# kjedrzejewski/video-cycle_gan-upscaling

Measured on AMD Instinct MI355X. Metric: upscaled frames/s (train step, G+D fwd+bwd) at 256->512, higher is better.
Workload: dtype f32; 1 GPU; C2: make_upscaler_orig((512,512,3),k=3,x2,res=9) + PatchGAN-70, batch 8/GPU, gan2 wiring, Wasserstein + pixel-MSE, faithful 3-call step incl. predict pass; global_batch=8, frame=256x256->512x512, parallelism=dp1, launch=hipGraph replay

## Files before the change

video-cycle_gan-upscaling_amd/csrc/conv_fwd.hip:

```cpp
#include "vcg_common.hpp"
#include <type_traits>

namespace {

struct ConvParams {
    const float* x;
    const float* w;
    float* y;
    const float* bias;
    const float* prelu;
    const float* residual;
    int n, cin, h, w_, cout, oh, ow, pad_top, pad_left;
    int tiles_x, tiles_y, co_blocks;
    int act;
    float alpha;
    int flip;
    int ws_t, ws_m, ws_k;
    float* stats;
};

template <int KH, int KW, int S, int CK, int XT>
struct ConvCfg {
    static constexpr int ROWS = 8;
    static constexpr int IH = (ROWS - 1) * S + KH;
    static constexpr int IW = (32 * XT - 1) * S + KW;
    static constexpr int PLANE = IH * IW;
    static constexpr int T = KH * KW;
    static constexpr int IN_ELEMS = CK * PLANE;
    static constexpr int W_ELEMS = CK * T * 64;
    static constexpr int IN_PT = (IN_ELEMS + 255) / 256;
    static constexpr int W_PT = (W_ELEMS + 255) / 256;
    static constexpr size_t LDS_BYTES = (size_t)(IN_ELEMS + W_ELEMS) * sizeof(float);
};

template <int XT>
__device__ __forceinline__ void conv_epilogue(const ConvParams& p, f32x16 (&acc)[2][2][XT], int n, int co0, int oy0, int ox0,
                                              int wv, int lane) {
    const int half = lane >> 5, l31 = lane & 31;
    const unsigned plane = (unsigned)(p.oh * p.ow), plane4 = 4u * plane, ow4 = 4u * (unsigned)p.ow;
    const int nch = p.cout - co0 < 64 ? p.cout - co0 : 64;
    const size_t blk = ((size_t)n * p.cout + co0) * plane;
    const size_t blk_bytes = (size_t)nch * plane * sizeof(float);
    const vcg_rsrc ry = make_rsrc(p.y + blk, blk_bytes);
    const vcg_rsrc rr = make_rsrc(p.residual ? p.residual + blk : nullptr, p.residual ? blk_bytes : 0);
    const bool is_prelu = p.act == VCG_ACT_PRELU;
    const vcg_rsrc rbias = make_rsrc(p.bias, p.bias ? (size_t)p.cout * sizeof(float) : 0);
    const vcg_rsrc rslope = make_rsrc(is_prelu ? p.prelu : nullptr, is_prelu ? (size_t)p.cout * sizeof(float) : 0);
    const float slope_u = (p.act == VCG_ACT_LRELU) ? p.alpha : 1.f;
    const unsigned chan4 = 4u * (unsigned)(co0 + 4 * half);

    const int oy = oy0 + wv * 2, ox = ox0 + l31;
    const unsigned base = (unsigned)(4 * half) * plane4 + (unsigned)oy * ow4 + 4u * (unsigned)ox;
    unsigned vo[2][XT];
#pragma unroll
    for (int rt = 0; rt < 2; ++rt)
#pragma unroll
        for (int xt = 0; xt < XT; ++xt)
            vo[rt][xt] = (oy + rt < p.oh && ox + xt * 32 < p.ow) ? base + (unsigned)rt * ow4 + 128u * xt : VCG_OOB;

    constexpr int RG = 8 / XT, NG = 32 / RG;
    auto emit = [&](auto res_tag) {
        constexpr bool RES = decltype(res_tag)::value;
        float rs[2][RG][2][XT];
        auto row_of = [](int g, int j) { const int q = g * RG + j, r = q & 15; return (q >> 4) * 32 + (r & 3) + 8 * (r >> 2); };
        auto load_res = [&](int g) {
#pragma unroll
            for (int j = 0; j < RG; ++j) {
                const unsigned srow = (unsigned)row_of(g, j) * plane4;
#pragma unroll
                for (int rt = 0; rt < 2; ++rt)
#pragma unroll
                    for (int xt = 0; xt < XT; ++xt) rs[g & 1][j][rt][xt] = buf_load(rr, __builtin_elementwise_add_sat(vo[rt][xt], srow));
            }
        };
        if (RES) load_res(0);
#pragma unroll
        for (int g = 0; g < NG; ++g) {
            float bv[RG], al[RG];
#pragma unroll
            for (int j = 0; j < RG; ++j) {
                bv[j] = buf_load(rbias, chan4 + 4u * (unsigned)row_of(g, j));
                const float pa = buf_load(rslope, chan4 + 4u * (unsigned)row_of(g, j));
                al[j] = is_prelu ? pa : slope_u;
            }
            if (RES && g + 1 < NG) load_res(g + 1);
#pragma unroll
            for (int j = 0; j < RG; ++j) {
                const int q = g * RG + j;
                const unsigned srow = (unsigned)row_of(g, j) * plane4;
#pragma unroll
                for (int rt = 0; rt < 2; ++rt) {
#pragma unroll
                    for (int xt = 0; xt < XT; ++xt) {
                        float v = acc[q >> 4][rt][xt][q & 15] + bv[j];
                        v = v >= 0.f ? v : v * al[j];
                        if (RES) v += rs[g & 1][j][rt][xt];
                        buf_store(ry, __builtin_elementwise_add_sat(vo[rt][xt], srow), v);
                    }
                }
            }
        }
    };
    if (p.residual) emit(std::true_type{}); else emit(std::false_type{});
}

template <int XT>
__device__ __forceinline__ void conv_stats_epilogue(const ConvParams& p, f32x16 (&acc)[2][2][XT], float* smem, int rec, int co0, int oy0, int ox0,
                                                    int wv, int lane, int tid) {
    const int half = lane >> 5, l31 = lane & 31;
    float sv[32], sq[32];
#pragma unroll
    for (int mt = 0; mt < 2; ++mt)
#pragma unroll
        for (int r = 0; r < 16; ++r) {
            float a = 0.f, b = 0.f;
#pragma unroll
            for (int rt = 0; rt < 2; ++rt)
#pragma unroll
                for (int xt = 0; xt < XT; ++xt) {
                    const bool ok = oy0 + wv * 2 + rt < p.oh && ox0 + l31 + xt * 32 < p.ow;
                    const float v = ok ? acc[mt][rt][xt][r] : 0.f;
                    a += v;
                    b = fmaf(v, v, b);
                }
            sv[mt * 16 + r] = a;
            sq[mt * 16 + r] = b;
        }
    const float ts = half_wave_reduce_scatter32(sv, l31), tq = half_wave_reduce_scatter32(sq, l31);
    const int ch = (l31 >> 4) * 32 + (l31 & 3) + 8 * ((l31 & 15) >> 2) + 4 * half;
    __syncthreads();
    smem[(0 * 4 + wv) * 64 + ch] = ts;
    smem[(1 * 4 + wv) * 64 + ch] = tq;
    __syncthreads();
    if (tid < 128) {
        const int st = tid >> 6, c = tid & 63;
        const float t = (smem[(st * 4 + 0) * 64 + c] + smem[(st * 4 + 1) * 64 + c]) + (smem[(st * 4 + 2) * 64 + c] + smem[(st * 4 + 3) * 64 + c]);
        if (co0 + c < p.cout) p.stats[((size_t)rec * 2 + st) * p.cout + co0 + c] = t;
    }
}

template <int KH, int KW, int S, int CK, int XT, bool STATS = false>
__global__ __launch_bounds__(256, (KH >= 9 ? 1 : 2)) void conv_fwd_kernel(const ConvParams p) {
    using C = ConvCfg<KH, KW, S, CK, XT>;
    extern __shared__ __attribute__((aligned(16))) float smem[];
    float* s_in = smem;
    float* s_w = smem + C::IN_ELEMS;

    const int tid = threadIdx.x, lane = tid & 63, wv = tid >> 6;
    const int half = lane >> 5, l31 = lane & 31;
    int b = blockIdx.x;
    const int cb = b % p.co_blocks; b /= p.co_blocks;
    const int tx = b % p.tiles_x;   b /= p.tiles_x;
    const int ty = b % p.tiles_y;   b /= p.tiles_y;
    const int n = b;
    const int ox0 = tx * 32 * XT, oy0 = ty * C::ROWS, co0 = cb * 64;
    const int gy0 = oy0 * S - p.pad_top, gx0 = ox0 * S - p.pad_left;
    const float* xn = p.x + (size_t)n * p.cin * p.h * p.w_;

    float rin[C::IN_PT], rw[C::W_PT];

    const int hw = p.h * p.w_;
    const int wvu = __builtin_amdgcn_readfirstlane(wv);
    const unsigned wcol = 4u * (unsigned)(co0 + lane < p.cout ? co0 + lane : p.cout - 1);
    const size_t wbytes = (size_t)C::T * p.cin * p.cout * sizeof(float);

    auto in_rsrc = [&](int ci0) { return make_rsrc(xn + (size_t)ci0 * hw, (size_t)(p.cin - ci0) * hw * sizeof(float)); };
    auto load_w = [&](int ci0) {
        const vcg_rsrc rwt = make_rsrc(p.w + (size_t)ci0 * p.cout, wbytes - (size_t)ci0 * p.cout * sizeof(float));
#pragma unroll
        for (int i = 0; i < C::W_PT; ++i) {
            const int q = wvu + 4 * i;
            const int t = q % C::T, ci = q / C::T;
            const int tap = p.flip ? (C::T - 1 - t) : t;
            rw[i] = buf_load(rwt, 4u * (unsigned)((tap * p.cin + ci) * p.cout) + wcol);
        }
    };
    load_w(0);
    __builtin_amdgcn_sched_barrier(0);

    unsigned in_off[C::IN_PT];
    {
        constexpr int Q1 = 256 / C::PLANE, R1 = 256 % C::PLANE, QR = R1 / C::IW, RC = R1 % C::IW;
        const vcg_rsrc rx = in_rsrc(0);
        const unsigned w4 = 4u * (unsigned)p.w_, hw4 = 4u * (unsigned)hw;
        const unsigned step = (unsigned)Q1 * hw4 + (unsigned)QR * w4 + 4u * RC;
        const unsigned col_wrap = w4 - 4u * C::IW, row_wrap = hw4 - (unsigned)C::IH * w4;
        int ci = tid / C::PLANE, r = (tid % C::PLANE) / C::IW, c = (tid % C::PLANE) % C::IW;
        unsigned off = (unsigned)ci * hw4 + (unsigned)(gy0 + r) * w4 + 4u * (unsigned)(gx0 + c);
#pragma unroll
        for (int i = 0; i < C::IN_PT; ++i) {
            const bool in_tile = (i + 1) * 256 <= C::IN_ELEMS || ci < CK;
            const bool ok = in_tile && (unsigned)(gy0 + r) < (unsigned)p.h && (unsigned)(gx0 + c) < (unsigned)p.w_;
            in_off[i] = ok ? off : VCG_OOB;
            rin[i] = buf_load(rx, in_off[i]);
            __builtin_amdgcn_sched_barrier(0);
            c += RC;
            const bool cw = c >= C::IW;
            c -= cw ? C::IW : 0;
            r += QR + (cw ? 1 : 0);
            const bool rwr = r >= C::IH;
            r -= rwr ? C::IH : 0;
            ci += Q1 + (rwr ? 1 : 0);
            off += step + (cw ? col_wrap : 0u) + (rwr ? row_wrap : 0u);
        }
    }
    auto load_chunk = [&](int ci0) {
        const vcg_rsrc rx = in_rsrc(ci0);
#pragma unroll
        for (int i = 0; i < C::IN_PT; ++i) rin[i] = buf_load(rx, in_off[i]);
        load_w(ci0);
    };
    auto store_chunk = [&]() {
#pragma unroll
        for (int i = 0; i < C::IN_PT; ++i) {
            const int e = tid + i * 256;
            if (e < C::IN_ELEMS) s_in[e] = rin[i];
        }
#pragma unroll
        for (int i = 0; i < C::W_PT; ++i) {
            const int e = tid + i * 256;
            if (e < C::W_ELEMS) s_w[e] = rw[i];
        }
    };

    f32x16 acc[2][2][XT];
#pragma unroll
    for (int i = 0; i < 2; ++i)
#pragma unroll
        for (int j = 0; j < 2; ++j)
#pragma unroll
            for (int x = 0; x < XT; ++x)
#pragma unroll
                for (int r = 0; r < 16; ++r) acc[i][j][x][r] = 0.f;

    const float* bbase = s_in + half * C::PLANE + (wv * 2 * S) * C::IW + l31 * S;
    const float* abase = s_w + half * C::T * 64 + l31;

    const int nchunks = (p.cin + CK - 1) / CK;
    for (int c = 0; c < nchunks; ++c) {
        __syncthreads();
        store_chunk();
        __syncthreads();
        if (c + 1 < nchunks) load_chunk((c + 1) * CK);
        constexpr int NTAP = (CK / 2) * C::T;
        auto rd = [&](int q, float (&a)[2], float (&b)[2][XT]) {
            const int cp = q / C::T, t = q % C::T, ky = t / KW, kx = t % KW;
            a[0] = abase[(cp * 2 * C::T + t) * 64];
            a[1] = abase[(cp * 2 * C::T + t) * 64 + 32];
#pragma unroll
            for (int xt = 0; xt < XT; ++xt) {
                b[0][xt] = bbase[cp * 2 * C::PLANE + ky * C::IW + kx + xt * 32 * S];
                b[1][xt] = bbase[cp * 2 * C::PLANE + (S + ky) * C::IW + kx + xt * 32 * S];
            }
        };
        float a_[2][2], b_[2][2][XT];
        rd(0, a_[0], b_[0]);
#pragma unroll
        for (int q = 0; q < NTAP; ++q) {
            const int cur = q & 1, nxt = cur ^ 1;
            if (q + 1 < NTAP) rd(q + 1, a_[nxt], b_[nxt]);
#pragma unroll
            for (int xt = 0; xt < XT; ++xt) {
                acc[0][0][xt] = mfma32(a_[cur][0], b_[cur][0][xt], acc[0][0][xt]);
                acc[0][1][xt] = mfma32(a_[cur][0], b_[cur][1][xt], acc[0][1][xt]);
                acc[1][0][xt] = mfma32(a_[cur][1], b_[cur][0][xt], acc[1][0][xt]);
                acc[1][1][xt] = mfma32(a_[cur][1], b_[cur][1][xt], acc[1][1][xt]);
            }
            if (q + 1 < NTAP) __builtin_amdgcn_sched_group_barrier(0x100, 1 + 2 * XT, 0);
            __builtin_amdgcn_sched_group_barrier(0x008, 4 * XT, 0);
        }
    }

    conv_epilogue<XT>(p, acc, n, co0, oy0, ox0, wv, lane);
    if (STATS) conv_stats_epilogue<XT>(p, acc, smem, (n * p.tiles_y + ty) * p.tiles_x + tx, co0, oy0, ox0, wv, lane, tid);
}

template <int KH, int KW, int S>
struct C3Cfg {
    static constexpr int ROWS = 8;
    static constexpr int IH = (ROWS - 1) * S + KH;
    static constexpr int IW = 31 * S + KW;
    static constexpr int PLANE = IH * IW;
    static constexpr int T = KH * KW;
    static constexpr int KT = 3 * T;
    static constexpr int NP = (KT + 1) / 2;
    static constexpr int IN_ELEMS = 3 * PLANE;
    static constexpr int W_ROWS = 2 * NP;
    static constexpr int W_ELEMS = W_ROWS * 64;
    static constexpr int IN_PT = (IN_ELEMS + 255) / 256;
    static constexpr int W_PT = W_ELEMS / 256;
    static constexpr size_t LDS_BYTES = (size_t)(IN_ELEMS + W_ELEMS) * sizeof(float);
    static constexpr int off(int k) { return (k / T) * PLANE + ((k % T) / KW) * IW + (k % T) % KW; }
    static constexpr int D_ROW = IW - (KW - 1);
    static constexpr int D_CH = PLANE - (KH - 1) * IW - (KW - 1);
};

template <int KH, int KW, int S>
__global__ __launch_bounds__(256, 2) void conv_c3_kernel(const ConvParams p) {
    using C = C3Cfg<KH, KW, S>;
    extern __shared__ __attribute__((aligned(16))) float smem[];
    float* s_in = smem;
    float* s_w = smem + C::IN_ELEMS;

    const int tid = threadIdx.x, lane = tid & 63, wv = tid >> 6;
    const int half = lane >> 5, l31 = lane & 31;
    int b = blockIdx.x;
    const int cb = b % p.co_blocks; b /= p.co_blocks;
    const int tx = b % p.tiles_x;   b /= p.tiles_x;
    const int ty = b % p.tiles_y;   b /= p.tiles_y;
    const int n = b;
    const int ox0 = tx * 32, oy0 = ty * C::ROWS, co0 = cb * 64;
    const int gy0 = oy0 * S - p.pad_top, gx0 = ox0 * S - p.pad_left;
    const float* xn = p.x + (size_t)n * p.cin * p.h * p.w_;

#pragma unroll
    for (int i = 0; i < C::IN_PT; ++i) {
        const int e = tid + i * 256;
        if (e < C::IN_ELEMS) {
            const int ci = e / C::PLANE, rem = e % C::PLANE;
            const int r = rem / C::IW, c = rem % C::IW;
            const int gy = gy0 + r, gx = gx0 + c;
            const bool ok = ci < p.cin && gy >= 0 && gy < p.h && gx >= 0 && gx < p.w_;
            const float v = xn[ok ? (ci * p.h + gy) * p.w_ + gx : 0];
            s_in[e] = ok ? v : 0.f;
        }
    }
#pragma unroll 4
    for (int i = 0; i < C::W_PT; ++i) {
        const int e = tid + i * 256;
        const int m = e & 63, k = e >> 6;
        const int ci = k / C::T, t = k % C::T;
        const int tap = p.flip ? (C::T - 1 - t) : t;
        const bool ok = k < C::KT && ci < p.cin && co0 + m < p.cout;
        const float v = p.w[ok ? (tap * p.cin + ci) * p.cout + co0 + m : 0];
        s_w[e] = ok ? v : 0.f;
    }
    __syncthreads();

    f32x16 acc[2][2][1];
#pragma unroll
    for (int i = 0; i < 2; ++i)
#pragma unroll
        for (int j = 0; j < 2; ++j)
#pragma unroll
            for (int r = 0; r < 16; ++r) acc[i][j][0][r] = 0.f;

    const float* b0p = s_in + (wv * 2 * S) * C::IW + l31 * S;
    const float* bb1 = b0p + half * 1;
    const float* bb2 = b0p + half * C::D_ROW;
    const float* bb3 = b0p + half * C::D_CH;
    const float* abase = s_w + half * 64 + l31;
#pragma unroll
    for (int pr = 0; pr < C::NP; ++pr) {
        constexpr int dummy = 0; (void)dummy;
        const int k0 = 2 * pr, k1 = 2 * pr + 1;
        const int o0 = C::off(k0);
        const int d = (k1 < C::KT) ? (C::off(k1) - o0) : 1;
        const float* bb = (d == 1) ? bb1 : (d == C::D_ROW ? bb2 : bb3);
        const float a0 = abase[k0 * 64];
        const float a1 = abase[k0 * 64 + 32];
        const float v0 = bb[o0];
        const float v1 = bb[o0 + S * C::IW];
        acc[0][0][0] = mfma32(a0, v0, acc[0][0][0]);
        acc[0][1][0] = mfma32(a0, v1, acc[0][1][0]);
        acc[1][0][0] = mfma32(a1, v0, acc[1][0][0]);
        acc[1][1][0] = mfma32(a1, v1, acc[1][1][0]);
    }
    conv_epilogue<1>(p, acc, n, co0, oy0, ox0, wv, lane);
}

template <int KH, int KW, int CK>
struct SmallCfg {
    static constexpr int ROWS = 8;
    static constexpr int XW = 64;
    static constexpr int OUTW = XW - (KW - 1);
    static constexpr int IH = ROWS + KH - 1;
    static constexpr int PLANE = IH * XW;
    static constexpr int IN_ELEMS = CK * PLANE;
    static constexpr int W_ELEMS = CK * KH * 32;
    static constexpr int IN_PT = (IN_ELEMS + 255) / 256;
    static constexpr int W_PT = (W_ELEMS + 255) / 256;
    static constexpr int PST = XW + 1;
    static constexpr int SCRATCH = 4 * 32 * PST;
    static constexpr int LDS_ELEMS = (IN_ELEMS + W_ELEMS) > SCRATCH ? (IN_ELEMS + W_ELEMS) : SCRATCH;
    static constexpr size_t LDS_BYTES = (size_t)LDS_ELEMS * sizeof(float);
};

template <int KH, int KW, int CK>
__global__ __launch_bounds__(256) void conv_smallm_kernel(const ConvParams p) {
    using C = SmallCfg<KH, KW, CK>;
    extern __shared__ __attribute__((aligned(16))) float smem[];
    float* s_in = smem;
    float* s_w = smem + C::IN_ELEMS;

    const int tid = threadIdx.x, lane = tid & 63, wv = tid >> 6;
    const int half = lane >> 5, l31 = lane & 31;
    int b = blockIdx.x;
    const int tx = b % p.tiles_x; b /= p.tiles_x;
    const int ty = b % p.tiles_y; b /= p.tiles_y;
    const int n = b;
    const int ox0 = tx * C::OUTW, oy0 = ty * C::ROWS;
    const int gy0 = oy0 - p.pad_top, gx0 = ox0 - p.pad_left;
    const float* xn = p.x + (size_t)n * p.cin * p.h * p.w_;
    const int mrows = p.cout * KW;

    float rin[C::IN_PT], rw[C::W_PT];
    const int wvu = __builtin_amdgcn_readfirstlane(tid >> 6);
    const int gx = gx0 + lane;
    const bool col_ok = gx >= 0 && gx < p.w_;
    const int gxc = min(max(gx, 0), p.w_ - 1);
    const int hw = p.h * p.w_;
    const vcg_rsrc rx = make_rsrc(xn, (size_t)p.cin * hw * sizeof(float));
    const vcg_rsrc rwt = make_rsrc(p.w, (size_t)KH * KW * p.cin * p.cout * sizeof(float));
    auto load_chunk = [&](int ci0) {
#pragma unroll
        for (int i = 0; i < C::IN_PT; ++i) {
            const int q = wvu + 4 * i;
            const int r = q % C::IH, ci = q / C::IH;
            const int gy = gy0 + r, ch = ci0 + ci;
            const bool ok = col_ok && ch < p.cin && gy >= 0 && gy < p.h;
            rin[i] = buf_load(rx, ok ? 4u * (unsigned)(ch * hw + gy * p.w_ + gxc) : VCG_OOB);
        }
#pragma unroll
        for (int i = 0; i < C::W_PT; ++i) {
            const int e = tid + i * 256;
            const int mi = e & 31, q = e >> 5;
            const int ky = q % KH, ci = q / KH;
            const int ch = ci0 + ci;
            const bool ok = e < C::W_ELEMS && ch < p.cin && mi < mrows;
            const int mch = mi / KW, kx = mi % KW;
            int tap = ky * KW + kx;
            if (p.flip) tap = KH * KW - 1 - tap;
            rw[i] = buf_load(rwt, ok ? 4u * (unsigned)(tap * p.ws_t + mch * p.ws_m + ch * p.ws_k) : VCG_OOB);
        }
    };
    auto store_chunk = [&]() {
#pragma unroll
        for (int i = 0; i < C::IN_PT; ++i) {
            const int e = tid + i * 256;
            if (e < C::IN_ELEMS) s_in[e] = rin[i];
        }
#pragma unroll
        for (int i = 0; i < C::W_PT; ++i) {
            const int e = tid + i * 256;
            if (e < C::W_ELEMS) s_w[e] = rw[i];
        }
    };

    f32x16 acc[2][2];
#pragma unroll
    for (int i = 0; i < 2; ++i)
#pragma unroll
        for (int j = 0; j < 2; ++j)
#pragma unroll
            for (int r = 0; r < 16; ++r) acc[i][j][r] = 0.f;

    const float* bbase = s_in + half * C::PLANE + (wv * 2) * C::XW + l31;
    const float* abase = s_w + half * KH * 32 + l31;

    const int nchunks = (p.cin + CK - 1) / CK;
    load_chunk(0);
    for (int c = 0; c < nchunks; ++c) {
        __syncthreads();
        store_chunk();
        __syncthreads();
        if (c + 1 < nchunks) load_chunk((c + 1) * CK);
#pragma unroll
        for (int cp = 0; cp < CK / 2; ++cp) {
#pragma unroll
            for (int ky = 0; ky < KH; ++ky) {
                const float a = abase[(cp * 2 * KH + ky) * 32];
                const float b00 = bbase[cp * 2 * C::PLANE + ky * C::XW];
                const float b01 = bbase[cp * 2 * C::PLANE + ky * C::XW + 32];
                const float b10 = bbase[cp * 2 * C::PLANE + (ky + 1) * C::XW];
                const float b11 = bbase[cp * 2 * C::PLANE + (ky + 1) * C::XW + 32];
                acc[0][0] = mfma32(a, b00, acc[0][0]);
                acc[0][1] = mfma32(a, b01, acc[0][1]);
                acc[1][0] = mfma32(a, b10, acc[1][0]);
                acc[1][1] = mfma32(a, b11, acc[1][1]);
            }
        }
    }

    float* s_p = smem + wv * 32 * C::PST;
#pragma unroll
    for (int rt = 0; rt < 2; ++rt) {
        __syncthreads();
#pragma unroll
        for (int xt = 0; xt < 2; ++xt)
#pragma unroll
            for (int r = 0; r < 16; ++r) s_p[mfma_row(r, lane) * C::PST + xt * 32 + l31] = acc[rt][xt][r];
        __syncthreads();
        const int oy = oy0 + wv * 2 + rt;
        const int ox = ox0 + lane;
        if (lane < C::OUTW && oy < p.oh && ox < p.ow) {
            for (int mch = 0; mch < p.cout; ++mch) {
                float v = 0.f;
#pragma unroll
                for (int kx = 0; kx < KW; ++kx) v += s_p[(mch * KW + kx) * C::PST + lane + kx];
                const float bv = p.bias ? p.bias[mch] : 0.f;
                const float al = (p.act == VCG_ACT_PRELU) ? p.prelu[mch] : p.alpha;
                const size_t idx = (((size_t)n * p.cout + mch) * p.oh + oy) * p.ow + ox;
                v = apply_act(v + bv, p.act, al);
                if (p.residual) v += p.residual[idx];
                p.y[idx] = v;
            }
        }
    }
}

template <int K>
__global__ __launch_bounds__(256) void conv_cout1_kernel(const ConvParams p) {
    __shared__ float red[4][64];
    const int tid = threadIdx.x, xl = tid & 63;
    const int cg = __builtin_amdgcn_readfirstlane(tid >> 6);
    int b = blockIdx.x;
    const int seg = b % p.tiles_x; b /= p.tiles_x;
    const int oy = b % p.oh;
    const int n = b / p.oh;
    const int ox = seg * 64 + xl, gx0 = ox - p.pad_left, gy0 = oy - p.pad_top;
    const int hw = p.h * p.w_;
    const vcg_rsrc rx = make_rsrc(p.x + (size_t)n * p.cin * hw, (size_t)p.cin * hw * sizeof(float));
    unsigned coff[K];
#pragma unroll
    for (int kx = 0; kx < K; ++kx) coff[kx] = (unsigned)(gx0 + kx) < (unsigned)p.w_ ? 4u * (unsigned)(gx0 + kx) : VCG_OOB;
    float acc = 0.f;
#pragma unroll 1
    for (int c = cg; c < p.cin; c += 4) {
        float wr[K * K];
#pragma unroll
        for (int t = 0; t < K * K; ++t) wr[t] = p.w[(p.flip ? K * K - 1 - t : t) * p.ws_t + c * p.ws_k];
#pragma unroll
        for (int ky = 0; ky < K; ++ky) {
            const int gy = gy0 + ky;
            const bool rok = (unsigned)gy < (unsigned)p.h;
            const unsigned rbase = 4u * (unsigned)(c * hw + gy * p.w_);
#pragma unroll
            for (int kx = 0; kx < K; ++kx) acc += buf_load(rx, rok && coff[kx] != VCG_OOB ? rbase + coff[kx] : VCG_OOB) * wr[ky * K + kx];
        }
    }
    red[cg][xl] = acc;
    __syncthreads();
    if (cg == 0 && ox < p.ow) {
        float v = ((red[0][xl] + red[1][xl]) + (red[2][xl] + red[3][xl])) + (p.bias ? p.bias[0] : 0.f);
        if (p.act == VCG_ACT_LRELU) v = v >= 0.f ? v : v * p.alpha;
        else if (p.act == VCG_ACT_TANH) v = tanhf(v);
        const size_t o = ((size_t)n * p.oh + oy) * p.ow + ox;
        if (p.residual) v += p.residual[o];
        p.y[o] = v;
    }
}

template <int K>
int launch_cout1(ConvParams p, hipStream_t st) {
    p.tiles_x = ceil_div(p.ow, 64);
    const long grid = (long)p.tiles_x * p.oh * p.n;
    if (grid <= 0 || grid > 0x7fffffffL) return VCG_E_SHAPE;
    hipLaunchKernelGGL(conv_cout1_kernel<K>, dim3((unsigned)grid), dim3(256), 0, st, p);
    VCG_LAUNCH_CHECK();
    return VCG_OK;
}

template <typename Kern>
int launch_with_lds(Kern kern, int grid, size_t lds, const ConvParams& p, hipStream_t st) {
    if (int e = vcg_allow_dyn_lds(reinterpret_cast<const void*>(kern), lds)) return e;
    hipLaunchKernelGGL(kern, dim3(grid), dim3(256), lds, st, p);
    VCG_LAUNCH_CHECK();
    return VCG_OK;
}

bool conv_block_fits(int oh, int ow, int ck, int h, int w) {
    const unsigned long long lim = 0xFFFFFFE0ull;
    return 64ull * oh * ow * sizeof(float) < lim && (unsigned long long)ck * h * w * sizeof(float) < lim;
}

template <int KH, int KW, int S, int CK, int XT>
int launch_conv(ConvParams p, hipStream_t st) {
    using C = ConvCfg<KH, KW, S, CK, XT>;
    if (!conv_block_fits(p.oh, p.ow, CK, p.h, p.w_)) return VCG_E_UNSUPPORTED;
    p.tiles_x = ceil_div(p.ow, 32 * XT);
    p.tiles_y = ceil_div(p.oh, C::ROWS);
    p.co_blocks = ceil_div(p.cout, 64);
    const long grid = (long)p.tiles_x * p.tiles_y * p.co_blocks * p.n;
    if (grid <= 0 || grid > 0x7fffffffL) return VCG_E_SHAPE;
    if (p.stats) {
        if constexpr ((KH == 3 && KW == 3 && S <= 2) || (KH == 4 && KW == 4 && S <= 2))
            return launch_with_lds(conv_fwd_kernel<KH, KW, S, CK, XT, true>, (int)grid, C::LDS_BYTES, p, st);
        else
            return VCG_E_UNSUPPORTED;
    }
    return launch_with_lds(conv_fwd_kernel<KH, KW, S, CK, XT>, (int)grid, C::LDS_BYTES, p, st);
}

template <int KH, int KW, int S>
int launch_c3(ConvParams p, hipStream_t st) {
    using C = C3Cfg<KH, KW, S>;
    if (!conv_block_fits(p.oh, p.ow, 3, p.h, p.w_)) return VCG_E_UNSUPPORTED;
    p.tiles_x = ceil_div(p.ow, 32);
    p.tiles_y = ceil_div(p.oh, C::ROWS);
    p.co_blocks = ceil_div(p.cout, 64);
    const long grid = (long)p.tiles_x * p.tiles_y * p.co_blocks * p.n;
    if (grid <= 0 || grid > 0x7fffffffL) return VCG_E_SHAPE;
    return launch_with_lds(conv_c3_kernel<KH, KW, S>, (int)grid, C::LDS_BYTES, p, st);
}

template <int KH, int KW, int CK>
int launch_smallm(ConvParams p, hipStream_t st) {
    using C = SmallCfg<KH, KW, CK>;
    p.tiles_x = ceil_div(p.ow, C::OUTW);
    p.tiles_y = ceil_div(p.oh, C::ROWS);
    p.co_blocks = 1;
    const long grid = (long)p.tiles_x * p.tiles_y * p.n;
    if (grid <= 0 || grid > 0x7fffffffL) return VCG_E_SHAPE;
    return launch_with_lds(conv_smallm_kernel<KH, KW, CK>, (int)grid, C::LDS_BYTES, p, st);
}

}

int vcg_internal_conv9_rowchain(const float* x, const float* w, float* y, int n, int cin, int h, int wd, int cout, const float* bias, int act,
                                int ws_t, int ws_m, int ws_k, hipStream_t st);

int vcg_internal_conv(const float* x, const float* w, float* y, int n, int cin, int h, int wd, int cout,
                      int oh, int ow, int kh, int kw, int stride, int pad_top, int pad_left, int flip,
                      const vcg_epilogue* ep, int smallm, int ws_t, int ws_m, int ws_k, hipStream_t st, float* stats) {
    ConvParams p{};
    p.x = x; p.w = w; p.y = y; p.stats = stats;
    if (stats && (smallm || cin <= 3)) return VCG_E_UNSUPPORTED;
    p.bias = ep ? ep->bias : nullptr;
    p.prelu = ep ? ep->prelu_alpha : nullptr;
    p.residual = ep ? ep->residual : nullptr;
    p.act = ep ? ep->act : VCG_ACT_NONE;
    p.alpha = ep ? ep->act_alpha : 0.f;
    if (p.act == VCG_ACT_PRELU && p.prelu == nullptr) return VCG_E_NULL;
    p.n = n; p.cin = cin; p.h = h; p.w_ = wd; p.cout = cout; p.oh = oh; p.ow = ow;
    p.pad_top = pad_top; p.pad_left = pad_left; p.flip = flip;
    p.ws_t = ws_t; p.ws_m = ws_m; p.ws_k = ws_k;
    if (n <= 0 || cin <= 0 || cout <= 0 || oh <= 0 || ow <= 0) return VCG_E_SHAPE;
    if (smallm) {
        if (stride != 1 || cout * kw > 32) return VCG_E_UNSUPPORTED;
        if (kh == 9 && kw == 9 && !flip && pad_top == 4 && pad_left == 4 && oh == h && ow == wd && !p.prelu && !p.residual) {
            const int rc = vcg_internal_conv9_rowchain(x, w, y, n, cin, h, wd, cout, p.bias, p.act, ws_t, ws_m, ws_k, st);
            if (rc != VCG_E_UNSUPPORTED) return rc;
        }
        if (cout == 1 && cin >= 64 && kh == kw && ws_m == 1 && !p.prelu && (size_t)cin * h * wd * 4 <= 0xFFFFFFE0u) {
            if (kh == 3) return launch_cout1<3>(p, st);
            if (kh == 4) return launch_cout1<4>(p, st);
            if (kh == 5) return launch_cout1<5>(p, st);
        }
        if (kh == 9 && kw == 9) return launch_smallm<9, 9, 8>(p, st);
        if (kh == 4 && kw == 4) return launch_smallm<4, 4, 8>(p, st);
        if (kh == 3 && kw == 3) return launch_smallm<3, 3, 8>(p, st);
        if (kh == 5 && kw == 5) return launch_smallm<5, 5, 8>(p, st);
        return VCG_E_UNSUPPORTED;
    }
    if (p.act == VCG_ACT_TANH) return VCG_E_UNSUPPORTED;
    if (cin <= 3) {
        if (kh == 9 && kw == 9 && stride == 1) return launch_c3<9, 9, 1>(p, st);
        if (kh == 3 && kw == 3 && stride == 1) return launch_c3<3, 3, 1>(p, st);
        if (kh == 4 && kw == 4 && stride == 2) return launch_c3<4, 4, 2>(p, st);
        if (kh == 5 && kw == 5 && stride == 1) return launch_c3<5, 5, 1>(p, st);
    }
    const bool wide = ow > 32;
    if (kh == 3 && kw == 3 && stride == 1) return wide ? launch_conv<3, 3, 1, 8, 2>(p, st) : launch_conv<3, 3, 1, 8, 1>(p, st);
    if (kh == 3 && kw == 3 && stride == 2) return launch_conv<3, 3, 2, 8, 1>(p, st);
    if (kh == 4 && kw == 4 && stride == 1) return launch_conv<4, 4, 1, 8, 1>(p, st);
    if (kh == 4 && kw == 4 && stride == 2) return launch_conv<4, 4, 2, 4, 1>(p, st);
    if (kh == 5 && kw == 5 && stride == 1) return launch_conv<5, 5, 1, 8, 1>(p, st);
    if (kh == 5 && kw == 5 && stride == 2) return launch_conv<5, 5, 2, 4, 1>(p, st);
    if (kh == 5 && kw == 5 && stride == 3) return launch_conv<5, 5, 3, 4, 1>(p, st);
    if (kh == 9 && kw == 9 && stride == 1) return launch_conv<9, 9, 1, 4, 1>(p, st);
    if (stride == 1) {
        if (kh == 1 && kw == 1) return launch_conv<1, 1, 1, 8, 1>(p, st);
        if (kh == 1 && kw == 3) return launch_conv<1, 3, 1, 8, 1>(p, st);
        if (kh == 3 && kw == 1) return launch_conv<3, 1, 1, 8, 1>(p, st);
        if (kh == 1 && kw == 5) return launch_conv<1, 5, 1, 8, 1>(p, st);
        if (kh == 5 && kw == 1) return launch_conv<5, 1, 1, 8, 1>(p, st);
        if (kh == 1 && kw == 7) return launch_conv<1, 7, 1, 8, 1>(p, st);
        if (kh == 7 && kw == 1) return launch_conv<7, 1, 1, 8, 1>(p, st);
    }
    return VCG_E_UNSUPPORTED;
}
```

Measured before the change: 134.2 frames/s.

## Make 3-channel conv a persistent kernel with double-buffered input tiles

Turns the cin=3 conv kernel into a persistent grid sized to twice the CU count. Each block walks tiles in a strided loop and prefetches the next tile's halo into registers while running MFMAs on the current LDS buffer, then stores it into a second LDS buffer. Weights are loaded once per block through buffer loads, and LDS reads are software-pipelined with scheduling barriers. This removes per-block launch and weight-reload overhead and hides global load latency, at the cost of doubled LDS for input and lower parallelism when there are few tiles.

New measurement: 136.1 frames/s, median of 6. 1.4% higher.

```diff
diff --git a/video-cycle_gan-upscaling_amd/csrc/conv_fwd.hip b/video-cycle_gan-upscaling_amd/csrc/conv_fwd.hip
--- a/video-cycle_gan-upscaling_amd/csrc/conv_fwd.hip
+++ b/video-cycle_gan-upscaling_amd/csrc/conv_fwd.hip
@@ -289,7 +289,9 @@
     static constexpr int W_ELEMS = W_ROWS * 64;
     static constexpr int IN_PT = (IN_ELEMS + 255) / 256;
     static constexpr int W_PT = W_ELEMS / 256;
-    static constexpr size_t LDS_BYTES = (size_t)(IN_ELEMS + W_ELEMS) * sizeof(float);
+    static constexpr int IN_BUF = IN_ELEMS + 4;
+    static constexpr size_t LDS_BYTES = (size_t)(2 * IN_BUF + W_ELEMS) * sizeof(float);
+    static_assert(IW < 256 && W_ELEMS % 256 == 0, "packed (row, column) of a halo element; whole weight rows per wave");
     static constexpr int off(int k) { return (k / T) * PLANE + ((k % T) / KW) * IW + (k % T) % KW; }
     static constexpr int D_ROW = IW - (KW - 1);
     static constexpr int D_CH = PLANE - (KH - 1) * IW - (KW - 1);
@@ -300,73 +302,144 @@
     using C = C3Cfg<KH, KW, S>;
     extern __shared__ __attribute__((aligned(16))) float smem[];
     float* s_in = smem;
-    float* s_w = smem + C::IN_ELEMS;
+    float* s_w = smem + 2 * C::IN_BUF;
 
     const int tid = threadIdx.x, lane = tid & 63, wv = tid >> 6;
     const int half = lane >> 5, l31 = lane & 31;
-    int b = blockIdx.x;
-    const int cb = b % p.co_blocks; b /= p.co_blocks;
-    const int tx = b % p.tiles_x;   b /= p.tiles_x;
-    const int ty = b % p.tiles_y;   b /= p.tiles_y;
-    const int n = b;
-    const int ox0 = tx * 32, oy0 = ty * C::ROWS, co0 = cb * 64;
-    const int gy0 = oy0 * S - p.pad_top, gx0 = ox0 * S - p.pad_left;
-    const float* xn = p.x + (size_t)n * p.cin * p.h * p.w_;
-
-#pragma unroll
-    for (int i = 0; i < C::IN_PT; ++i) {
-        const int e = tid + i * 256;
-        if (e < C::IN_ELEMS) {
-            const int ci = e / C::PLANE, rem = e % C::PLANE;
-            const int r = rem / C::IW, c = rem % C::IW;
-            const int gy = gy0 + r, gx = gx0 + c;
-            const bool ok = ci < p.cin && gy >= 0 && gy < p.h && gx >= 0 && gx < p.w_;
-            const float v = xn[ok ? (ci * p.h + gy) * p.w_ + gx : 0];
-            s_in[e] = ok ? v : 0.f;
-        }
-    }
-#pragma unroll 4
-    for (int i = 0; i < C::W_PT; ++i) {
-        const int e = tid + i * 256;
-        const int m = e & 63, k = e >> 6;
-        const int ci = k / C::T, t = k % C::T;
-        const int tap = p.flip ? (C::T - 1 - t) : t;
-        const bool ok = k < C::KT && ci < p.cin && co0 + m < p.cout;
-        const float v = p.w[ok ? (tap * p.cin + ci) * p.cout + co0 + m : 0];
-        s_w[e] = ok ? v : 0.f;
-    }
-    __syncthreads();
-
-    f32x16 acc[2][2][1];
-#pragma unroll
-    for (int i = 0; i < 2; ++i)
-#pragma unroll
-        for (int j = 0; j < 2; ++j)
-#pragma unroll
-            for (int r = 0; r < 16; ++r) acc[i][j][0][r] = 0.f;
-
+    const int nblk = p.co_blocks, step = (int)gridDim.x / nblk;
+    const int cb = (int)blockIdx.x % nblk, co0 = cb * 64;
+    int t = (int)blockIdx.x / nblk;
+    const int tiles = p.n * p.tiles_y * p.tiles_x;
+    if (t >= tiles) return;
+    int tx = t % p.tiles_x, ty = (t / p.tiles_x) % p.tiles_y, n = t / (p.tiles_x * p.tiles_y);
+    const int dtx = step % p.tiles_x, dty = (step / p.tiles_x) % p.tiles_y, dn = step / (p.tiles_x * p.tiles_y);
+
+    constexpr bool KEEP = C::IN_PT <= 8;
+    const int hw = p.h * p.w_;
+    const unsigned w4 = 4u * (unsigned)p.w_, hw4 = 4u * (unsigned)hw;
+    const size_t img_bytes = (size_t)p.cin * hw * sizeof(float);
+    auto decode = [&](int tid_, int i, unsigned& rel_, unsigned& rc_) {
+        const int e = tid_ + i * 256;
+        const int ci = e / C::PLANE, rem = e % C::PLANE;
+        const int r = rem / C::IW, c = rem % C::IW;
+        rel_ = (unsigned)ci * hw4 + (unsigned)r * w4 + 4u * (unsigned)c;
+        rc_ = (unsigned)(r << 8 | c);
+    };
+    unsigned rel[KEEP ? C::IN_PT : 1], rc[KEEP ? C::IN_PT : 1];
+    if constexpr (KEEP) {
+#pragma unroll
+        for (int i = 0; i < C::IN_PT; ++i) {
+            decode(tid, i, rel[i], rc[i]);
+            asm volatile("" : "+v"(rc[i]));
+        }
+    }
+    const bool last_live = tid + (C::IN_PT - 1) * 256 < C::IN_ELEMS;
+    float rin[C::IN_PT];
+    auto load_tile = [&](int n_, int ty_, int tx_) {
+        const int gy0 = ty_ * C::ROWS * S - p.pad_top, gx0 = tx_ * 32 * S - p.pad_left;
+        const vcg_rsrc rx = make_rsrc(p.x + (size_t)n_ * p.cin * hw, img_bytes);
+        const unsigned tb = (unsigned)gy0 * w4 + 4u * (unsigned)gx0;
+        int tid_t = tid;
+        if constexpr (!KEEP) asm volatile("" : "+v"(tid_t));
+#pragma unroll
+        for (int i = 0; i < C::IN_PT; ++i) {
+            unsigned rl, q;
+            if constexpr (KEEP) { rl = rel[i]; q = rc[i]; } else decode(tid_t, i, rl, q);
+            bool ok = (unsigned)(gy0 + (int)(q >> 8)) < (unsigned)p.h && (unsigned)(gx0 + (int)(q & 255u)) < (unsigned)p.w_;
+            if (i == C::IN_PT - 1) ok = ok && last_live;
+            rin[i] = buf_load(rx, ok ? tb + rl : VCG_OOB);
+        }
+    };
+    auto store_tile = [&](float* buf) {
+#pragma unroll
+        for (int i = 0; i < C::IN_PT; ++i) {
+            const int e = tid + i * 256;
+            if (e < C::IN_ELEMS) buf[e] = rin[i];
+        }
+    };
+    load_tile(n, ty, tx);
+
+    {
+        const vcg_rsrc rwt = make_rsrc(p.w, (size_t)C::T * p.cin * p.cout * sizeof(float));
+        const int wvu = __builtin_amdgcn_readfirstlane(wv);
+        const unsigned col = co0 + lane < p.cout ? 4u * (unsigned)(co0 + lane) : VCG_OOB;
+        float rw[C::W_PT];
+#pragma unroll
+        for (int i = 0; i < C::W_PT; ++i) {
+            const int k = wvu + 4 * i;
+            const int ci = k / C::T, tt = k % C::T;
+            const int tap = p.flip ? (C::T - 1 - tt) : tt;
+            const unsigned row = (k < C::KT && ci < p.cin) ? 4u * (unsigned)((tap * p.cin + ci) * p.cout) : VCG_OOB;
+            rw[i] = buf_load(rwt, __builtin_elementwise_add_sat(col, row));
+        }
+        if (tid < 8) s_in[(tid >> 2) * C::IN_BUF + C::IN_ELEMS + (tid & 3)] = 0.f;
+#pragma unroll
+        for (int i = 0; i < C::W_PT; ++i) s_w[tid + i * 256] = rw[i];
+    }
+    store_tile(s_in);
+    lds_barrier();
+
+    const float* abase = s_w + half * 64 + l31;
     const float* b0p = s_in + (wv * 2 * S) * C::IW + l31 * S;
-    const float* bb1 = b0p + half * 1;
-    const float* bb2 = b0p + half * C::D_ROW;
-    const float* bb3 = b0p + half * C::D_CH;
-    const float* abase = s_w + half * 64 + l31;
-#pragma unroll
-    for (int pr = 0; pr < C::NP; ++pr) {
-        constexpr int dummy = 0; (void)dummy;
-        const int k0 = 2 * pr, k1 = 2 * pr + 1;
-        const int o0 = C::off(k0);
-        const int d = (k1 < C::KT) ? (C::off(k1) - o0) : 1;
-        const float* bb = (d == 1) ? bb1 : (d == C::D_ROW ? bb2 : bb3);
-        const float a0 = abase[k0 * 64];
-        const float a1 = abase[k0 * 64 + 32];
-        const float v0 = bb[o0];
-        const float v1 = bb[o0 + S * C::IW];
-        acc[0][0][0] = mfma32(a0, v0, acc[0][0][0]);
-        acc[0][1][0] = mfma32(a0, v1, acc[0][1][0]);
-        acc[1][0][0] = mfma32(a1, v0, acc[1][0][0]);
-        acc[1][1][0] = mfma32(a1, v1, acc[1][1][0]);
-    }
-    conv_epilogue<1>(p, acc, n, co0, oy0, ox0, wv, lane);
+    int cur = 0;
+    for (;;) {
+        const bool more = step < tiles - t;
+        const int n0 = n, oy0 = ty * C::ROWS, ox0 = tx * 32;
+        if (more) {
+            t += step;
+            tx += dtx;
+            const int cx = tx >= p.tiles_x ? 1 : 0;
+            tx -= cx ? p.tiles_x : 0;
+            ty += dty + cx;
+            const int cy = ty >= p.tiles_y ? 1 : 0;
+            ty -= cy ? p.tiles_y : 0;
+            n += dn + cy;
+            load_tile(n, ty, tx);
+        }
+
+        f32x16 acc[2][2][1];
+#pragma unroll
+        for (int i = 0; i < 2; ++i)
+#pragma unroll
+            for (int j = 0; j < 2; ++j)
+#pragma unroll
+                for (int r = 0; r < 16; ++r) acc[i][j][0][r] = 0.f;
+
+        const float* b0 = b0p + cur * C::IN_BUF;
+        const float* bb1 = b0 + half * 1;
+        const float* bb2 = b0 + half * C::D_ROW;
+        const float* bb3 = b0 + half * C::D_CH;
+        auto rd = [&](int pr, float (&f)[4]) {
+            const int k0 = 2 * pr, k1 = 2 * pr + 1;
+            const int o0 = C::off(k0);
+            const int d = (k1 < C::KT) ? (C::off(k1) - o0) : 1;
+            const float* bb = (d == 1) ? bb1 : (d == C::D_ROW ? bb2 : bb3);
+            f[0] = abase[k0 * 64];
+            f[1] = abase[k0 * 64 + 32];
+            f[2] = bb[o0];
+            f[3] = bb[o0 + S * C::IW];
+        };
+        float f_[2][4];
+        rd(0, f_[0]);
+#pragma unroll
+        for (int pr = 0; pr < C::NP; ++pr) {
+            const float(&f)[4] = f_[pr & 1];
+            if (pr + 1 < C::NP) rd(pr + 1, f_[(pr & 1) ^ 1]);
+            acc[0][0][0] = mfma32(f[0], f[2], acc[0][0][0]);
+            acc[0][1][0] = mfma32(f[0], f[3], acc[0][1][0]);
+            acc[1][0][0] = mfma32(f[1], f[2], acc[1][0][0]);
+            acc[1][1][0] = mfma32(f[1], f[3], acc[1][1][0]);
+            if (pr + 1 < C::NP) __builtin_amdgcn_sched_group_barrier(0x100, 4, 0);
+            __builtin_amdgcn_sched_group_barrier(0x008, 4, 0);
+        }
+        if (more) {
+            store_tile(s_in + (cur ^ 1) * C::IN_BUF);
+            lds_barrier();
+        }
+        conv_epilogue<1>(p, acc, n0, co0, oy0, ox0, wv, lane);
+        if (!more) break;
+        cur ^= 1;
+    }
 }
 
 template <int KH, int KW, int CK>
@@ -592,6 +665,15 @@
     return launch_with_lds(conv_fwd_kernel<KH, KW, S, CK, XT>, (int)grid, C::LDS_BYTES, p, st);
 }
 
+int device_cu_count() {
+    static const int cus = [] {
+        int dev = 0, v = 0;
+        if (hipGetDevice(&dev) != hipSuccess || hipDeviceGetAttribute(&v, hipDeviceAttributeMultiprocessorCount, dev) != hipSuccess) return 0;
+        return v;
+    }();
+    return cus;
+}
+
 template <int KH, int KW, int S>
 int launch_c3(ConvParams p, hipStream_t st) {
     using C = C3Cfg<KH, KW, S>;
@@ -599,8 +681,13 @@
     p.tiles_x = ceil_div(p.ow, 32);
     p.tiles_y = ceil_div(p.oh, C::ROWS);
     p.co_blocks = ceil_div(p.cout, 64);
-    const long grid = (long)p.tiles_x * p.tiles_y * p.co_blocks * p.n;
-    if (grid <= 0 || grid > 0x7fffffffL) return VCG_E_SHAPE;
+    const long tiles = (long)p.tiles_x * p.tiles_y * p.co_blocks * p.n;
+    if (tiles <= 0 || tiles > 0x7fffffffL) return VCG_E_SHAPE;
+    const int cus = device_cu_count();
+    if (cus <= 0) return VCG_E_UNSUPPORTED;
+    long grid = tiles < 2L * cus ? tiles : 2L * cus;
+    grid -= grid % p.co_blocks;
+    if (grid < p.co_blocks) grid = p.co_blocks;
     return launch_with_lds(conv_c3_kernel<KH, KW, S>, (int)grid, C::LDS_BYTES, p, st);
 }
 
```
